# resibots/limbo

Measured on AMD Instinct MI355X. Metric: GP compute()+log_lik evaluations/sec at N=4096 D=6 fp64, higher is better.
Workload: dtype f64

## Files before the change

### limbo_amd/csrc/gemm.hip

```cpp
#include "dev.h"
#include <hip/hip_ext.h>
#include <cstdio>
#include <cstdint>
#include <cstdlib>
#include <map>
#include <mutex>
#include <tuple>
#include <vector>
#include <algorithm>

#ifdef GEMM_TIMING
__device__ long long g_gemm_ts[16];
#define GTS(i) do { if (threadIdx.x == 0 && blockIdx.x == 0 && lwg == (int)blockIdx.x) g_gemm_ts[i] = clock64(); } while (0)
__device__ long long g_gemm64_ts[24];
#define GTS64(i) do { if (threadIdx.x == 0 && blockIdx.x == 0 && lwg == (int)blockIdx.x) g_gemm64_ts[i] = clock64(); } while (0)
#else
#define GTS(i) do { } while (0)
#define GTS64(i) do { } while (0)
#endif
#ifdef GEMM_TIMING
#define GTS64_(i) GTS64(i)
#endif
#include "gemm_glds64.h"
#ifndef GEMM_ABL
// ... 127 lines not shown
    const double* Ap = AK ? g.A + kbeg + row0 * g.lda : g.A + row0 + kbeg * g.lda;
    const double* Bp = BK ? g.B + kbeg + col0 * g.ldb : g.B + col0 + kbeg * g.ldb;
    const int64_t a_kstep = AK ? (int64_t)BKT : (int64_t)BKT * g.lda;
    const int64_t b_kstep = BK ? (int64_t)BKT : (int64_t)BKT * g.ldb;
    const int64_t mrows = g.m - row0, ncols = g.n - col0;
    const int mr = (int)(mrows < TM ? mrows : TM), nc = (int)(ncols < TN ? ncols : TN);

    double acc[RA][RB];
#pragma unroll
    for (int a = 0; a < RA; ++a)
#pragma unroll
        for (int b = 0; b < RB; ++b)
            acc[a][b] = 0.0;

    using WT = WaveTileC<RA, RB>;
    double* Cw = g.C + (col0 + wn) * g.ldc + row0 + wm;
    const int rlim = mr - wm < WT::R ? mr - wm : WT::R, clim = nc - wn < WT::CN ? nc - wn : WT::CN;
    const bool live = rlim > 0 && clim > 0;
    constexpr bool CPRE = (NBUF == 1);
    double cv[WT::NIT];
    if (CPRE && live && g.overwrite != 1)
        WT::load(cv, Cw, g.ldc, rlim, clim, lane);

    SA sa;
    SB sb;
    int64_t kleft = kend - kbeg;
    if (kleft > 0) {
        const int kl = (int)(kleft < BKT ? kleft : BKT);
        sa.template load<true>(Ap, g.lda, mr, kl);
        sb.template load<false>(Bp, g.ldb, nc, kl);
        sa.store(lds[0]);
        sb.store(lds[0] + SA::ELEMS);
    }
    __syncthreads();
    int buf = 0;
    for (int64_t k0 = kbeg; k0 < kend; k0 += BKT) {
#if GEMM_ABL != 1
        const bool more = (NBUF == 2) && (k0 + BKT < kend);
#endif
#if GEMM_ABL == 1
        const bool more = false;
#endif
        if (more) {
            Ap += a_kstep;
            Bp += b_kstep;
            const int64_t kleft2 = kend - k0 - BKT;
            const int kl = (int)(kleft2 < BKT ? kleft2 : BKT);
            sa.template load<true>(Ap, g.lda, mr, kl);
            sb.template load<false>(Bp, g.ldb, nc, kl);
        }
        const double* As = lds[buf];
        const double* Bs = lds[buf] + SA::ELEMS;
#pragma unroll
        for (int ks = 0; ks < BKT; ks += 4) {
            double af[RA], bf[RB];
#pragma unroll
            for (int x = 0; x < RA; ++x)
                af[x] = SA::at(As, arow + 16 * x, ks + kq);
#pragma unroll
            for (int x = 0; x < RB; ++x)
                bf[x] = SB::at(Bs, bcol + 4 * x, ks + kq);
#pragma unroll
            for (int n = 0; n < RB; ++n)
#pragma unroll
                for (int m = 0; m < RA; ++m)
#if GEMM_ABL == 2
                    acc[m][n] += af[m] * bf[n] * (ks == 0 && m == 0 && n == 0 ? 1.0 : 0.0);
#else
                    acc[m][n] = mfma4(af[m], bf[n], acc[m][n]);
#endif
        }
        if (NBUF == 2) {
            if (more) {
                sa.store(lds[buf ^ 1]);
                sb.store(lds[buf ^ 1] + SA::ELEMS);
            }
            __syncthreads();
            buf ^= 1;
        }
    }

    static_assert(4 * WT::SCRATCH <= NBUF * (SA::ELEMS + SB::ELEMS), "transposition scratch must fit in the operand stages");
    if (!CPRE && live && g.overwrite != 1)
        WT::load(cv, Cw, g.ldc, rlim, clim, lane);
    if (NBUF == 1)
        __syncthreads();
    if (live)
        WT::store(acc, cv, &lds[0][0] + wave * WT::SCRATCH, Cw, g.ldc, rlim, clim, g.overwrite, lane);
}

template <typename K>
static void launch_k_named(const char* name, K kern_single, K kern_batched, dim3 grid, dim3 block, hipStream_t s, const GemmArgs& g0)
{
    GemmArgs g = g0;
    g.bt = g_batch.bt;
    grid.z = (unsigned)g_batch.G;
    K kern = g.bt ? kern_batched : kern_single;
    if (g.stop_event)
        GPE_LAUNCH_STOP(name, kern, grid, block, 0, s, (hipEvent_t)g.stop_event, g);
    else
        GPE_LAUNCH_NAMED(name, kern, grid, block, 0, s, g);
}
#define launch_k(ks, ...) launch_k_named(#ks, ks, __VA_ARGS__)
template <int TM, int TN, int BKT, int NBUF>
static void launch_tile(hipStream_t s, const GemmArgs& g0)
{
    GemmArgs g = g0;
    const int tiles_m = (int)((g.m + TM - 1) / TM), tiles_n = (int)((g.n + TN - 1) / TN);
    int64_t tiles = (int64_t)tiles_m * tiles_n;
    if (g.tri) {
        int fold = 1;
        const int nsup = (tiles_n + 1) / 2;
        for (int sc = 0; sc < nsup; ++sc) {
            const int t2 = tiles_n - 1 - sc;
            int len = tiles_m - first_live_tile<TM, TN>(g, sc);
            if (t2 != sc)
                len += tiles_m - first_live_tile<TM, TN>(g, t2);
            fold = len > fold ? len : fold;
        }
        g.fold_len = fold;
        tiles = (int64_t)nsup * fold;
    }
    dim3 grid((unsigned)tiles), block(256);
    if (!g.a_kmajor && !g.b_kmajor)
        launch_k(k_gemm4<TM, TN, BKT, NBUF, false, false>, k_gemm4<TM, TN, BKT, NBUF, false, false, true>, grid, block, s, g);
    else if (!g.a_kmajor && g.b_kmajor)
        launch_k(k_gemm4<TM, TN, BKT, NBUF, false, true>, k_gemm4<TM, TN, BKT, NBUF, false, true, true>, grid, block, s, g);
    else if (g.a_kmajor && !g.b_kmajor)
        launch_k(k_gemm4<TM, TN, BKT, NBUF, true, false>, k_gemm4<TM, TN, BKT, NBUF, true, false, true>, grid, block, s, g);
    else
        launch_k(k_gemm4<TM, TN, BKT, NBUF, true, true>, k_gemm4<TM, TN, BKT, NBUF, true, true, true>, grid, block, s, g);
}


template <int TM, int TN, int WM, int WN, int BKT, int NST, int EPC = 0, int MINB = 1, bool BATCH = false>
__global__ __launch_bounds__(WM* WN * 64, MINB) void k_gemm_glds(GemmArgs g_)
{
    GemmArgs gb;
    if (BATCH) {
        gb = g_;
        gemm_rebase(gb);
    }
    const GemmArgs& g = BATCH ? gb : g_;
    static_assert(TM == 128 && TN == 128, "one k-row of an operand tile = one 1 KiB glds instruction");
    constexpr int NWV = WM * WN;
    constexpr int SA = TM + 16, SB = TN + 16;
    constexpr int STAGE = BKT * (SA + SB);
    constexpr int RA = TM / WM / 16, RB = TN / WN / 4;
    constexpr int LPW = 2 * BKT / NWV;
    __shared__ __attribute__((aligned(16))) double lds[NST * STAGE];

    const int tiles_m = (int)((g.m + TM - 1) / TM);
    const int tiles_n = (int)((g.n + TN - 1) / TN);
    if (g.rhs_rows > 0)
        gemm_rhs_rows<64 * NWV, MINB == 1>(g, g.rhs_rows, (int)gridDim.x, lds);
    for (int lwg = blockIdx.x; lwg < g.total; lwg += gridDim.x) {
    int wg = lwg;
    {
        const int nwg = g.total;
        const int q = nwg / 8, r = nwg % 8, xcd = wg % 8, idx = wg / 8;
        wg = (xcd < r ? xcd * (q + 1) : r * (q + 1) + (xcd - r) * q) + idx;
    }
    int ti, tj;
    if (g.tile_map) {
        const int pk = g.tile_map[lwg];
        if (pk < 0)
            continue;
        ti = pk & 0xffff;
        tj = pk >> 16;
    }
    else if (g.tri) {
        const int sc = wg / g.fold_len;
        int rr = wg % g.fold_len;
        const int t0 = first_live_tile<TM, TN>(g, sc), c0 = tiles_m - t0;
        if (rr < c0) {
            tj = sc;
            ti = t0 + rr;
        }
        else {
            tj = tiles_n - 1 - sc;
            const int t1 = first_live_tile<TM, TN>(g, tj);
            rr -= c0;
            if (tj == sc || rr >= tiles_m - t1)
                continue;
            ti = t1 + rr;
        }
    }
    else {
        ti = wg % tiles_m;
        tj = wg / tiles_m;
    }
    const int64_t row0 = (int64_t)ti * TM, col0 = (int64_t)tj * TN;
    const int64_t mrows = g.m - row0, ncols = g.n - col0;
    const int mr = (int)(mrows < TM ? mrows : TM), nc = (int)(ncols < TN ? ncols : TN);

    const int lane = threadIdx.x & 63;
    const int wave = __builtin_amdgcn_readfirstlane(threadIdx.x >> 6);
    const int wm = (wave % WM) * (TM / WM), wn = (wave / WM) * (TN / WN);
    const int arow = wm + (lane & 15), bcol = wn + (lane & 3), kq = lane >> 4;

    int ra = 2 * lane, rb = 2 * lane;
    {
        const int ma = (mr - 1) & ~1, mb = (nc - 1) & ~1;
        ra = ra < ma ? ra : ma;
        rb = rb < mb ? rb : mb;
    }
    const int64_t kbeg = g.ktri ? (row0 > col0 ? row0 : col0) : 0;
    const double* pa = g.A + row0 + ra + ((int64_t)wave + kbeg) * g.lda;
    const double* pb = g.B + col0 + rb + ((int64_t)wave + kbeg) * g.ldb;
    const int64_t astep = (int64_t)NWV * g.lda, bstep = (int64_t)NWV * g.ldb;

    auto issue = [&](int stage) {
        double* sa = lds + stage * STAGE + wave * SA;
        double* sb = lds + stage * STAGE + BKT * SA + wave * SB;
#pragma unroll
        for (int q = 0; q < BKT / NWV; ++q) {
            __builtin_amdgcn_global_load_lds(pa, (lds_void_t*)(sa + q * NWV * SA), 16, 0, 0);
            __builtin_amdgcn_global_load_lds(pb, (lds_void_t*)(sb + q * NWV * SB), 16, 0, 0);
            pa += astep;
            pb += bstep;
        }
    };

    double acc[RA][RB];
#pragma unroll
    for (int a = 0; a < RA; ++a)
#pragma unroll
        for (int b = 0; b < RB; ++b)
            acc[a][b] = 0.0;

    const int nk = (int)((g.k - kbeg) / BKT);
    GTS(0);
    issue(0);
    for (int t = 0; t < nk; ++t) {
        const int st = t % NST;
        if (t + 1 < nk) {
            issue((t + 1) % NST);
            asm volatile("s_waitcnt vmcnt(%0)" ::"n"(LPW) : "memory");
        }
        else
            asm volatile("s_waitcnt vmcnt(0)" ::: "memory");
        __builtin_amdgcn_s_barrier();
        if (t == 0)
            GTS(1);
        if (t == 1)
            GTS(2);
        if (t == 2)
            GTS(3);
        const double* As = lds + st * STAGE;
        const double* Bs = As + BKT * SA;
#pragma unroll
        for (int ks = 0; ks < BKT; ks += 4) {
            double af[RA], bf[RB];
#pragma unroll
            for (int x = 0; x < RA; ++x)
                af[x] = As[(ks + kq) * SA + arow + 16 * x];
#pragma unroll
            for (int x = 0; x < RB; ++x)
                bf[x] = Bs[(ks + kq) * SB + bcol + 4 * x];
#pragma unroll
            for (int n = 0; n < RB; ++n)
#pragma unroll
                for (int m = 0; m < RA; ++m)
                    acc[m][n] = mfma4(af[m], bf[n], acc[m][n]);
        }
        if (t == 1)
            GTS(6);
        asm volatile("s_waitcnt lgkmcnt(0)" ::: "memory");
        __builtin_amdgcn_s_barrier();
        if (t == 1)
            GTS(7);
    }
    GTS(4);

    {
        using WT = WaveTileC<RA, RB>;
        constexpr int SCR = EPC > 0 ? WT::SCRATCH / EPC : WT::SCRATCH;
        static_assert(NWV * SCR <= NST * STAGE, "transposition scratch must fit in the operand stages");
        double* Cw = g.C + (col0 + wn) * g.ldc + row0 + wm;
        const int rlim = mr - wm < WT::R ? mr - wm : WT::R, clim = nc - wn < WT::CN ? nc - wn : WT::CN;
        if (rlim > 0 && clim > 0) {
            if constexpr (EPC > 0)
                WT::template rmw_chunked<EPC>(acc, lds + wave * SCR, Cw, g.ldc, rlim, clim, g.overwrite, lane);
            else {
                double cv[WT::NIT];
                if (g.overwrite != 1)
                    WT::load(cv, Cw, g.ldc, rlim, clim, lane);
                WT::store(acc, cv, lds + wave * WT::SCRATCH, Cw, g.ldc, rlim, clim, g.overwrite, lane);
            }
        }
    }
    __syncthreads();
    GTS(5);
    }
}
#ifdef GEMM_TIMING
void dump_gemm_timing()
{
    {
        long long q[24];
        (void)hipMemcpyFromSymbol(q, HIP_SYMBOL(g_gemm64_ts), sizeof(q));
        printf("k_gemm_glds64 WG0 first tile, cycles: start->k-tile 0 begins %lld | k-tiles:", q[1] - q[0]);
        for (int t = 1; t < 16; ++t)
            printf(" %lld", q[1 + t] - q[t]);
        printf(" %lld | epilogue %lld | total %lld\n", q[17] - q[16], q[18] - q[17], q[18] - q[0]);
    }
    long long h[16];
    (void)hipMemcpyFromSymbol(h, HIP_SYMBOL(g_gemm_ts), sizeof(h));
    printf("k_gemm_glds WG0 first tile, cycles: prologue (first stage landed) %lld | k-tile 0 %lld | k-tile 1 %lld (mfma part %lld, closing barrier %lld) | whole k loop %lld | epilogue %lld | total %lld\n",
           h[1] - h[0], h[2] - h[1], h[3] - h[2], h[6] - h[2], h[7] - h[6], h[4] - h[1], h[5] - h[4], h[5] - h[0]);
    printf("  epilogue: issue 32 loads %lld | loads complete %lld | issue 32 stores %lld | stores complete %lld | tail %lld\n", h[8] - h[4],
           h[9] - h[8], h[10] - h[9], h[11] - h[10], h[5] - h[11]);
}
#endif

template <int BKT, int NST, int MINB, int NWV, bool BATCH = false>
__global__ __launch_bounds__(64 * NWV, MINB) void k_gemm_glds64(GemmArgs g_)
{
    GemmArgs gb;
    if (BATCH) {
        gb = g_;
        gemm_rebase(gb);
    }
    const GemmArgs& g = BATCH ? gb : g_;
    __shared__ __attribute__((aligned(16))) double lds[NST * Glds64Shape<BKT>::STAGE];
    gemm_glds64_body<BKT, NST, NWV>(g, lds, (int)blockIdx.x, (int)gridDim.x, false);
}

static void launch_glds64(hipStream_t s, const GemmArgs& g0)
{
    constexpr int TM = 64, TN = 64;
    GemmArgs g = g0;
    const int tiles_m = (int)((g.m + TM - 1) / TM), tiles_n = (int)((g.n + TN - 1) / TN);
    int64_t tiles = (int64_t)tiles_m * tiles_n;
    if (g.tri) {
        int fold = 1;
        const int nsup = (tiles_n + 1) / 2;
        for (int sc = 0; sc < nsup; ++sc) {
            const int t2 = tiles_n - 1 - sc;
            int len = tiles_m - first_live_tile<TM, TN>(g, sc);
            if (t2 != sc)
                len += tiles_m - first_live_tile<TM, TN>(g, t2);
            fold = len > fold ? len : fold;
        }
        g.fold_len = fold;
        tiles = (int64_t)nsup * fold;
    }
    g.total = (int)tiles;
    if ((int64_t)g.total * g_batch.G > 256)
        launch_k(k_gemm_glds64<16, 4, 2, 4>, k_gemm_glds64<16, 4, 2, 4, true>, dim3((unsigned)tiles), dim3(256), s, g);
    else
        launch_k(k_gemm_glds64<16, 4, 1, 8>, k_gemm_glds64<16, 4, 1, 8, true>, dim3((unsigned)tiles), dim3(512), s, g);
}

static bool glds_ok(const GemmArgs& g)
{
    return !g.a_kmajor && !g.b_kmajor && !g.ktri && g.k >= 32 && g.k % 32 == 0 && (g.lda % 2) == 0 && (g.ldb % 2) == 0
        && ((uintptr_t)g.A % 16) == 0 && ((uintptr_t)g.B % 16) == 0;
}

#define TRI_BAND 8
struct TriMapKey {
    int dev, tiles_m, tiles_n;
    int64_t off;
    bool operator<(const TriMapKey& o) const
    {
        return std::tie(dev, tiles_m, tiles_n, off) < std::tie(o.dev, o.tiles_m, o.tiles_n, o.off);
    }
};
static int tri_tile_map_host(const GemmArgs& g, std::vector<int>& tab)
{
    constexpr int TM = 128, TN = 128;
    const int tiles_m = (int)((g.m + TM - 1) / TM), tiles_n = (int)((g.n + TN - 1) / TN);
    std::vector<int> first(tiles_n);
    for (int tj = 0; tj < tiles_n; ++tj)
        first[tj] = first_live_tile<TM, TN>(g, tj);
    std::vector<int> seq;
    for (int r0 = 0; r0 < tiles_m; r0 += TRI_BAND) {
        const int r1 = std::min(tiles_m, r0 + TRI_BAND);
        for (int tj = 0; tj < tiles_n; ++tj)
            for (int ti = std::max(r0, first[tj]); ti < r1; ++ti)
                seq.push_back(ti | (tj << 16));
    }
    const int T = (int)seq.size(), q = T / 8, r = T % 8, slots = q + (r ? 1 : 0);
    tab.assign((size_t)slots * 8, -1);
    int pos = 0;
    for (int x = 0; x < 8; ++x) {
        const int len = q + (x < r ? 1 : 0);
        for (int i = 0; i < len; ++i)
            tab[(size_t)i * 8 + x] = seq[pos + i];
        pos += len;
    }
    return (int)tab.size();
}
int debug_tri_tile_map(int64_t m, int64_t n, int64_t grow0, int64_t gcol0, int* out, int cap)
{
    GemmArgs g{};
    g.m = m;
    g.n = n;
    g.tri = 1;
    g.grow0 = grow0;
    g.gcol0 = gcol0;
    std::vector<int> tab;
    const int len = tri_tile_map_host(g, tab);
    for (int i = 0; i < len && i < cap; ++i)
        out[i] = tab[i];
    return len;
}
static const int* tri_tile_map(const GemmArgs& g, int* total)
{
    static std::mutex mu;
    static std::map<TriMapKey, std::pair<int*, int>> cache;
    int dev = 0;
    (void)hipGetDevice(&dev);
    const TriMapKey key{dev, (int)((g.m + 127) / 128), (int)((g.n + 127) / 128), g.gcol0 - g.grow0};
    std::lock_guard<std::mutex> lk(mu);
    auto it = cache.find(key);
    if (it == cache.end()) {
        std::vector<int> tab;
        const int len = tri_tile_map_host(g, tab);
        int* d = nullptr;
        if (hipMalloc(&d, sizeof(int) * (size_t)len) != hipSuccess)
            return nullptr;
        if (hipMemcpy(d, tab.data(), sizeof(int) * (size_t)len, hipMemcpyHostToDevice) != hipSuccess) {
            (void)hipFree(d);
            return nullptr;
// ... 408 lines not shown
```

### limbo_amd/csrc/potrf_tail.hip

```cpp
#include "potrf_tile.h"
#include <array>
#include <map>
#include <mutex>
#include <vector>
#ifdef DIAG_TIMING
__device__ long long g_tail_ts[64][4];
__device__ long long g_tail_cyc[64][4];
#define TTS(c, i) do { if (threadIdx.x == 0 && (c) < 64) { g_tail_ts[(c)][(i)] = wall_clock64(); g_tail_cyc[(c)][(i)] = clock64(); } } while (0)
__device__ long long g_tail_ts2[64][12];
#define TTS2(x, on, i) do { if ((on) && threadIdx.x == 0 && ((x).R0 - (x).p0) / NB < 64) g_tail_ts2[((x).R0 - (x).p0) / NB][(i)] = wall_clock64(); } while (0)
#else
#define TTS(c, i) do { } while (0)
#define TTS2(x, on, i) do { } while (0)
#endif

struct TailArgs {
    double* A;
    int64_t lda, t0;
    int nt, nb;
    int nfull;
    int rhs_rows;
    double* Xt;
    int* info;
    double *LP, *SP, *LPn, *SPn;
// ... 348 lines not shown
    }
    __syncthreads();
    TTS2(x, true, 3);
    double y2[2][2] = {{0.0, 0.0}, {0.0, 0.0}};
    tri_solve32(T, 32, X22, wm, hn, lane, y2);
#pragma unroll
    for (int m = 0; m < 2; ++m)
#pragma unroll
        for (int n = 0; n < 2; ++n)
            Ys[(hn + 4 * n + dcol) * PS + wm + 16 * m + drow] = y2[m][n];
    __syncthreads();
    TTS2(x, true, 4);
    syrk40<32>(Ys, 0, wave, lane, a2v);
    syrk40_store_neg(Dl, wave, lane, a2v);
    {
        const int i = threadIdx.x & 63, kk0 = threadIdx.x >> 6;
#pragma unroll
        for (int q = 0; q < 4; ++q) {
            const int col = kk0 + 8 * q;
            __hip_atomic_store(pub + i + NB * (32 + col), Ys[col * PS + i], __ATOMIC_RELAXED, __HIP_MEMORY_SCOPE_AGENT);
        }
    }
#pragma unroll
    for (int m = 0; m < 2; ++m)
#pragma unroll
        for (int n = 0; n < 2; ++n)
            T[(32 + hn + 4 * n + dcol) * PS + wm + 16 * m + drow] = y2[m][n];
    TTS2(x, true, 5);
}

static __device__ __forceinline__ void tail_tile_solve(const P256& x, double* __restrict__ lds, const double (&own)[8],
                                                       const double* __restrict__ Sq, double* __restrict__ pub, const bool near)
{
    const int lane = threadIdx.x & 63, wave = __builtin_amdgcn_readfirstlane(threadIdx.x >> 6);
    const int wm = (wave & 1) * 32, wn = (wave >> 1) * 16;
    const int hn = tri_solve_cols(wave);
    const int crow = wm + (lane & 31), ccol = wn + (lane >> 5);
    const int drow = 4 * ((lane >> 2) & 3) + (lane >> 4), dcol = lane & 3;
    double* const T = lds + CH_T;
    double* const X11 = lds + CH_X11;
    double* const Ld = lds + CH_LD;
    double* const Ys = lds + CH_YS;
    double* const X22 = lds + CH_X22;
    const unsigned long long SENT = ~0ull;
    const unsigned long long* Sp = reinterpret_cast<const unsigned long long*>(Sq) + threadIdx.x;
#pragma unroll
    for (int it = 0; it < 8; ++it)
        T[(ccol + 2 * it) * PS + crow] = own[it];
    {
        unsigned long long xb[4];
#pragma unroll
        for (int q = 0; q < 4; ++q)
            xb[q] = __hip_atomic_load(Sp + 512 * q, __ATOMIC_RELAXED, POLL_FIRST_SCOPE);
        if (near)
            chain_watch<4>(Sp, xb, x.spin_limit, x.info);
        else {
            int spins = 0;
            while (xb[0] == SENT || xb[1] == SENT || xb[2] == SENT || xb[3] == SENT) {
                if (++spins > x.spin_limit) {
                    x.info[2] = 1;
                    break;
                }
                poll_one(Sq + 1023, x.spin_limit, x.info);
                poll_one(Sq + 1024 + 32 * 31, x.spin_limit, x.info);
#pragma unroll
                for (int q = 0; q < 4; ++q)
                    if (xb[q] == SENT)
                        xb[q] = __hip_atomic_load(Sp + 512 * q, __ATOMIC_RELAXED, __HIP_MEMORY_SCOPE_AGENT);
            }
        }
#pragma unroll
        for (int q = 0; q < 2; ++q) {
            const int e = threadIdx.x + 512 * q;
            X11[(e >> 5) * 34 + (e & 31)] = __longlong_as_double((long long)xb[q]);
            Ld[(e & 31) * 34 + (e >> 5)] = __longlong_as_double((long long)xb[2 + q]);
        }
    }
    __syncthreads();
    double y1[2][2] = {{0.0, 0.0}, {0.0, 0.0}};
    tri_solve32(T, 0, X11, wm, hn, lane, y1);
#pragma unroll
    for (int m = 0; m < 2; ++m)
#pragma unroll
        for (int n = 0; n < 2; ++n)
            Ys[(hn + 4 * n + dcol) * PS + wm + 16 * m + drow] = y1[m][n];
    __syncthreads();
    double u[2][2] = {{0.0, 0.0}, {0.0, 0.0}};
    mmk<true, 32, 2, 34>(Ys, 0, Ld, 0, wm, hn, lane, u);
#pragma unroll
    for (int m = 0; m < 2; ++m)
#pragma unroll
        for (int n = 0; n < 2; ++n) {
            double* t = T + (32 + hn + 4 * n + dcol) * PS + wm + 16 * m + drow;
            *t = *t - u[m][n];
            T[(hn + 4 * n + dcol) * PS + wm + 16 * m + drow] = y1[m][n];
        }
    {
        const int i = threadIdx.x & 63, kk0 = threadIdx.x >> 6;
#pragma unroll
        for (int q = 0; q < 4; ++q) {
            const int col = kk0 + 8 * q;
            __hip_atomic_store(pub + i + NB * col, Ys[col * PS + i], __ATOMIC_RELAXED, __HIP_MEMORY_SCOPE_AGENT);
        }
    }
    {
        unsigned long long xc[2];
        xc[0] = __hip_atomic_load(Sp + 2048, __ATOMIC_RELAXED, POLL_FIRST_SCOPE);
        xc[1] = __hip_atomic_load(Sp + 2048 + 512, __ATOMIC_RELAXED, POLL_FIRST_SCOPE);
        if (near)
            chain_watch<2>(Sp + 2048, xc, x.spin_limit, x.info);
        else {
            int spins = 0;
            while (xc[0] == SENT || xc[1] == SENT) {
                if (++spins > x.spin_limit) {
                    x.info[2] = 1;
                    break;
                }
                poll_one(Sq + 2048 + 1023, x.spin_limit, x.info);
                if (xc[0] == SENT)
                    xc[0] = __hip_atomic_load(Sp + 2048, __ATOMIC_RELAXED, __HIP_MEMORY_SCOPE_AGENT);
                if (xc[1] == SENT)
                    xc[1] = __hip_atomic_load(Sp + 2048 + 512, __ATOMIC_RELAXED, __HIP_MEMORY_SCOPE_AGENT);
            }
        }
        const int e0 = threadIdx.x, e1 = threadIdx.x + 512;
        X22[(e0 >> 5) * 34 + (e0 & 31)] = __longlong_as_double((long long)xc[0]);
        X22[(e1 >> 5) * 34 + (e1 & 31)] = __longlong_as_double((long long)xc[1]);
    }
    __syncthreads();
    double y2[2][2] = {{0.0, 0.0}, {0.0, 0.0}};
    tri_solve32(T, 32, X22, wm, hn, lane, y2);
#pragma unroll
    for (int m = 0; m < 2; ++m)
#pragma unroll
        for (int n = 0; n < 2; ++n)
            Ys[(hn + 4 * n + dcol) * PS + wm + 16 * m + drow] = y2[m][n];
    __syncthreads();
    {
        const int i = threadIdx.x & 63, kk0 = threadIdx.x >> 6;
#pragma unroll
        for (int q = 0; q < 4; ++q) {
            const int col = kk0 + 8 * q;
            __hip_atomic_store(pub + i + NB * (32 + col), Ys[col * PS + i], __ATOMIC_RELAXED, __HIP_MEMORY_SCOPE_AGENT);
        }
    }
#pragma unroll
    for (int m = 0; m < 2; ++m)
#pragma unroll
        for (int n = 0; n < 2; ++n)
            T[(32 + hn + 4 * n + dcol) * PS + wm + 16 * m + drow] = y2[m][n];
    __syncthreads();
}

static __device__ __forceinline__ void tail_body(const TailArgs& a, const int wgid, double* __restrict__ lds,
                                                 const KParams* __restrict__ kp = nullptr)
{
    const int lane = threadIdx.x & 63, wave = __builtin_amdgcn_readfirstlane(threadIdx.x >> 6);
    const int wm = (wave & 1) * 32, wn = (wave >> 1) * 16;
    const int crow = wm + (lane & 31), ccol = wn + (lane >> 5);
    int c = 0, b;
    if (a.order) {
        b = __builtin_amdgcn_readfirstlane(a.order[2 * wgid]);
        c = __builtin_amdgcn_readfirstlane(a.order[2 * wgid + 1]);
    }
    else {
        int id = wgid, colh = a.nb;
        while (id >= colh) {
            id -= colh;
            ++c;
            --colh;
        }
        b = c + id;
    }
    const int slot = tail_tile_id(a.nb, b, c);
    const bool mute = a.spin_limit < 0;
    P256 x;
    x.A = a.A;
    x.lda = a.lda;
    x.p0 = a.t0;
    x.R0 = a.t0 + (int64_t)NB * b;
    x.Xt = a.Xt;
    x.info = a.info;
    x.mute = mute;
    x.spin_limit = mute ? -a.spin_limit : a.spin_limit;
    x.nrows = b < a.nfull ? NB : a.rhs_rows;
    x.want_d = false;
    x.Bx = lds;
    x.T0 = lds + NB * XS;
    x.T1 = x.T0 + NB * PS;
    x.T2 = x.T1 + NB * PS;
    x.S22 = a.SP;
    x.HP = a.LP;
    double* const myslot = a.LP + (int64_t)slot * (NB * NB);
    {
        unsigned long long* nx = reinterpret_cast<unsigned long long*>(a.LPn + (int64_t)slot * (NB * NB));
#pragma unroll
        for (int q = 0; q < 8; ++q)
            nx[threadIdx.x + 512 * q] = ~0ull;
        if (b == c) {
            unsigned long long* ns = reinterpret_cast<unsigned long long*>(a.SPn + (int64_t)c * 3072);
#pragma unroll
            for (int q = 0; q < 6; ++q)
                ns[threadIdx.x + 512 * q] = ~0ull;
        }
    }
    if (b == c + 1 && b < a.nt)
        return;
    const int crc = crow < x.nrows ? crow : x.nrows - 1;
    double cv[8];
    if (kp) {
        tail_gen_tile(a, kp, x.R0 + crc, a.t0 + (int64_t)NB * c + ccol, cv);
        if (a.Al && b >= a.nfull && threadIdx.x < NB)
            for (int p = 0; p < a.P; ++p)
                reinterpret_cast<unsigned long long*>(a.Al)[a.t0 + (int64_t)NB * c + threadIdx.x + (int64_t)p * a.ldal] = ~0ull;
    }
    else {
#pragma unroll
        for (int it = 0; it < 8; ++it)
            cv[it] = a.A[x.R0 + crc + (a.t0 + (int64_t)NB * c + ccol + 2 * it) * a.lda];
    }
    if (b == c) {
        double* const Dl = lds + CH_D;
        double* const Ltb = lds + CH_AUX;
        double* const invd = Ltb + DIAG_LTB;
        DiagSync* const sy = reinterpret_cast<DiagSync*>(invd + NB);
        if (c > 0) {
            double cl[8];
            if (kp)
                tail_gen_tile(a, kp, x.R0 + crow, a.t0 + (int64_t)NB * (c - 1) + ccol, cl);
            else {
#pragma unroll
                for (int it = 0; it < 8; ++it)
                    cl[it] = a.A[x.R0 + crow + (a.t0 + (int64_t)NB * (c - 1) + ccol + 2 * it) * a.lda];
            }
            tail_chain_updates_and_crossing(a, x, lds, c, cl, cv);
            TTS(c, 1);
        }
        else {
#pragma unroll
            for (int it = 0; it < 8; ++it)
                Dl[crow * XS + ccol + 2 * it] = cv[it];
            diag_flow_init(sy);
        }
        __syncthreads();
        DiagEarly ea;
        ea.mute = mute;
        ea.S = a.SP + (int64_t)c * 3072;
        TTS(c, 2);
        diag_flow(Dl, Ltb, invd, sy, a.A + x.R0 + x.R0 * a.lda, a.lda, a.Xt + (int64_t)c * (NB * NB), a.info, x.R0, wave, lane,
                  invd + NB + 8, &ea);
        TTS(c, 3);
        if (c > 0) {
            __syncthreads();
            const int i = threadIdx.x & 63, kk0 = threadIdx.x >> 6;
            double* Ag = a.A + x.R0 + (a.t0 + (int64_t)NB * (c - 1)) * a.lda;
            const double* T = lds + CH_T;
#pragma unroll
            for (int q = 0; q < 8; ++q) {
                const int col = kk0 + 8 * q;
                Ag[i + (int64_t)col * a.lda] = T[col * PS + i];
            }
        }
        return;
    }
    PolledTile pa, pb;
    if (c > 0) {
        pa.issue(a.LP + (int64_t)tail_tile_id(a.nb, b, 0) * (NB * NB));
        pb.issue(a.LP + (int64_t)tail_tile_id(a.nb, c, 0) * (NB * NB));
    }
    double a2[2][4] = {{0.0, 0.0, 0.0, 0.0}, {0.0, 0.0, 0.0, 0.0}};
#pragma unroll 1
    for (int s = 0; s < c; ++s) {
        double* const opA = lds + (s & 1) * (2 * NB * PS);
        double* const opB = opA + NB * PS;
        pa.finish(a.LP + (int64_t)tail_tile_id(a.nb, b, s) * (NB * NB), x.spin_limit, x.info);
        pa.store(opA);
        pb.finish(a.LP + (int64_t)tail_tile_id(a.nb, c, s) * (NB * NB), x.spin_limit, x.info);
        pb.store(opB);
        if (s + 1 < c) {
            pa.issue(a.LP + (int64_t)tail_tile_id(a.nb, b, s + 1) * (NB * NB));
            pb.issue(a.LP + (int64_t)tail_tile_id(a.nb, c, s + 1) * (NB * NB));
        }
        __syncthreads();
        mm64<false>(opA, opB, wm, wn, lane, a2);
    }
    if (c > 0) {
        double a2r[8];
        wave_tile_to_rows(a2, a2r, lane);
#pragma unroll
        for (int it = 0; it < 8; ++it)
            cv[it] -= a2r[it];
        __syncthreads();
    }
    tail_tile_solve(x, lds, cv, a.SP + (int64_t)c * 3072, myslot, b - c <= 3);
    {
        const int i = threadIdx.x & 63, kk0 = threadIdx.x >> 6;
        double* Ag = a.A + x.R0 + (a.t0 + (int64_t)NB * c) * a.lda;
        const double* T = lds + CH_T;
        if (i < x.nrows) {
#pragma unroll
            for (int q = 0; q < 8; ++q) {
                const int col = kk0 + 8 * q;
                Ag[i + (int64_t)col * a.lda] = T[col * PS + i];
            }
        }
    }
}

__global__ __launch_bounds__(512) void k_tail(TailArgs a)
{
    __shared__ __attribute__((aligned(16))) double lds[TAIL_LDS_DOUBLES];
    tail_body(a, (int)blockIdx.x, lds);
}
__global__ __launch_bounds__(512) void k_tail_g(TailArgs a, KParams kp)
{
    __shared__ __attribute__((aligned(16))) double lds[TAIL_LDS_DOUBLES];
    tail_body(a, (int)blockIdx.x, lds, &kp);
}
__global__ __launch_bounds__(512) void k_tail_b(TailArgs a, const BatchTab* __restrict__ bt)
{
    __shared__ __attribute__((aligned(16))) double lds[TAIL_LDS_DOUBLES];
    const int G = bt->G, gp = (int)blockIdx.x % G;
    a.A = bt_rebase(bt, gp, a.A);
    a.Xt = bt_rebase(bt, gp, a.Xt);
    a.info = bt_rebase(bt, gp, a.info);
    a.LP = bt_rebase(bt, gp, a.LP);
    a.SP = bt_rebase(bt, gp, a.SP);
    a.LPn = bt_rebase(bt, gp, a.LPn);
    a.SPn = bt_rebase(bt, gp, a.SPn);
    if (a.Xg) {
        a.Xg = bt_rebase(bt, gp, a.Xg);
        a.Om = bt_rebase(bt, gp, a.Om);
        a.Al = bt_rebase(bt, gp, a.Al);
    }
    tail_body(a, (int)blockIdx.x / G, lds, a.Xg ? &bt->kp[gp] : nullptr);
}

__global__ __launch_bounds__(256) void k_ragged_partial(const double* __restrict__ A, int64_t ld, int m, int n, int64_t k, int kc,
                                                        double* __restrict__ part)
{
    __shared__ __attribute__((aligned(16))) double As[32][NB];
    const int li = threadIdx.x & 63, lk = threadIdx.x >> 6;
    const int ti = threadIdx.x & 15, tj = threadIdx.x >> 4;
    const int64_t k0 = (int64_t)blockIdx.x * kc, k1 = k0 + kc < k ? k0 + kc : k;
    double acc[4][4];
#pragma unroll
    for (int r = 0; r < 4; ++r)
#pragma unroll
        for (int c = 0; c < 4; ++c)
            acc[r][c] = 0.0;
    double nx[8];
    auto fetch = [&](int64_t kb) {
#pragma unroll
        for (int q = 0; q < 8; ++q) {
            const int kk = lk + 4 * q;
            nx[q] = (kb + kk < k1 && li < m) ? A[li + (kb + kk) * ld] : 0.0;
        }
    };
    fetch(k0);
    for (int64_t kb = k0; kb < k1; kb += 32) {
        __syncthreads();
#pragma unroll
        for (int q = 0; q < 8; ++q)
            As[lk + 4 * q][li] = nx[q];
        if (kb + 32 < k1)
            fetch(kb + 32);
        __syncthreads();
#pragma unroll 8
        for (int kk = 0; kk < 32; ++kk) {
            double a[4], b[4];
#pragma unroll
            for (int r = 0; r < 4; ++r) {
                a[r] = As[kk][4 * ti + r];
                b[r] = As[kk][4 * tj + r];
            }
#pragma unroll
            for (int r = 0; r < 4; ++r)
#pragma unroll
                for (int c = 0; c < 4; ++c)
                    acc[r][c] = fma(a[r], b[c], acc[r][c]);
        }
    }
    double* out = part + (int64_t)blockIdx.x * (NB * NB);
#pragma unroll
    for (int c = 0; c < 4; ++c)
#pragma unroll
        for (int r = 0; r < 4; ++r)
            out[4 * ti + r + NB * (4 * tj + c)] = acc[r][c];
}
#define RAGGED_MAX_G 32
__global__ __launch_bounds__(256) void k_ragged_fold(double* __restrict__ C, int64_t ldc, int m, int n, int G, const double* __restrict__ part)
{
    const int i = threadIdx.x & 63, j = 4 * (int)blockIdx.x + (threadIdx.x >> 6);
    if (i >= m || j >= n || i < j)
        return;
    double v[RAGGED_MAX_G];
#pragma unroll
    for (int g = 0; g < RAGGED_MAX_G; ++g)
        v[g] = g < G ? part[(int64_t)g * (NB * NB) + i + NB * j] : 0.0;
    double sum = 0.0;
#pragma unroll
    for (int g = 0; g < RAGGED_MAX_G; ++g)
        sum += v[g];
    C[i + (int64_t)j * ldc] -= sum;
}
int ragged_split(int64_t k, int64_t scratch_doubles, int* kc_out)
{
    if (k < 256 || scratch_doubles < 2 * NB * NB)
        return 0;
    int64_t G = k / 64;
    G = G > RAGGED_MAX_G ? RAGGED_MAX_G : G;
    G = G > scratch_doubles / (NB * NB) ? scratch_doubles / (NB * NB) : G;
    const int64_t kc = ((k + G - 1) / G + 31) / 32 * 32;
    G = (k + kc - 1) / kc;
    *kc_out = (int)kc;
    return (int)G;
}
__global__ __launch_bounds__(DIAG_THREADS) void k_ragged_finish(double* __restrict__ C, int64_t ldc, int jb, int P, int G,
                                                                const double* __restrict__ part, double* __restrict__ Lscr,
                                                                double* __restrict__ Xt, int* __restrict__ info, int64_t goff)
{
    __shared__ __attribute__((aligned(16))) double Ls[NB * XS];
    __shared__ __attribute__((aligned(16))) double Ltb[DIAG_LTB];
    __shared__ __attribute__((aligned(16))) double invd[NB];
    __shared__ DiagSync sy;
    __shared__ __attribute__((aligned(16))) double Xw[DIAG_XW_DOUBLES];
    __shared__ double Rr[NB * 65];
    const int lane = threadIdx.x & 63, w = __builtin_amdgcn_readfirstlane(threadIdx.x >> 6);
    const int m = jb + P;
    for (int e = threadIdx.x; e < NB * 65; e += DIAG_THREADS)
// ... 282 lines not shown
```

### limbo_amd/csrc/sweep2.hip

```cpp
#include "gemm_glds64.h"

#define NB 64
#define S2_PS 80
#define S2_MS 65

#ifdef S2_TIMING
__device__ long long g_s2_ts[256][6];
#define S2TS(i) do { if (threadIdx.x == 0) g_s2_ts[j][i] = wall_clock64(); } while (0)
#else
#define S2TS(i) do { } while (0)
#endif

__global__ __launch_bounds__(512) void k_trsv_bwd_m(const double* __restrict__ L, int64_t ld, int64_t N, const double* __restrict__ Xt_all,
                                                    const double* __restrict__ y, int64_t ysi, double* a, int* __restrict__ err,
                                                    const double* __restrict__ om, double* __restrict__ part)
{
    __shared__ __attribute__((aligned(16))) double lds[2 * NB * S2_PS];
    __shared__ double Mt[NB * S2_MS], M2t[NB * S2_MS];
    __shared__ double xs[NB], wj[NB], gj[NB], part_s[8 * NB];
    const int lane = threadIdx.x & 63, wv = threadIdx.x >> 6;
    const int wvu = __builtin_amdgcn_readfirstlane(wv);
    const int64_t nblk = (N + NB - 1) / NB;
    const int64_t j = flow_block_of(nblk, true);
    if (j < 0)
        return;
    const int64_t j0 = j * NB;
    const int jb = (int)((N - j0 < NB) ? N - j0 : NB);
    const double* Xt = Xt_all + j * (NB * NB);
    const unsigned long long SENT = ~0ull;
    S2TS(0);
    if (j + 1 < nblk) {
        double* As = lds;
        double* Bs = lds + NB * S2_PS;
        const int wm = (wvu & 1) * 32, wn = (wvu >> 1) * 16;
        const int ar = wm + (lane & 15), bc = wn + (lane & 3), kq = lane >> 4;
        const int drow = 4 * ((lane >> 2) & 3) + (lane >> 4), dcol = lane & 3;
#pragma unroll
        for (int q = 0; q < 8; ++q) {
            const int r = wvu + 8 * q;
            As[r * S2_PS + lane] = Xt[lane + NB * r];
        }
        for (int q2 = 1; q2 <= 2 && j + q2 < nblk; ++q2) {
            const int64_t t0 = (j + q2) * NB;
            const int tb = (int)((N - t0 < NB) ? N - t0 : NB);
            const int kc = lane < tb ? lane : tb - 1;
            const double km = lane < tb ? 1.0 : 0.0;
            if (q2 == 2)
                __syncthreads();
#pragma unroll
            for (int q = 0; q < 8; ++q) {
                const int r = wvu + 8 * q;
                const int rc = r < jb ? r : jb - 1;
                Bs[r * S2_PS + lane] = L[t0 + kc + (j0 + rc) * ld] * (r < jb ? km : 0.0);
            }
            __syncthreads();
            double acc[2][4] = {{0.0, 0.0, 0.0, 0.0}, {0.0, 0.0, 0.0, 0.0}};
#pragma unroll
            for (int ks = 0; ks < NB; ks += 4) {
                double af[2], bf[4];
#pragma unroll
                for (int x = 0; x < 2; ++x)
                    af[x] = As[(ks + kq) * S2_PS + ar + 16 * x];
#pragma unroll
                for (int x = 0; x < 4; ++x)
                    bf[x] = Bs[(ks + kq) * S2_PS + bc + 4 * x];
#pragma unroll
                for (int n = 0; n < 4; ++n)
#pragma unroll
                    for (int m = 0; m < 2; ++m)
                        acc[m][n] = mfma4(af[m], bf[n], acc[m][n]);
            }
            double* Md = q2 == 1 ? Mt : M2t;
#pragma unroll
            for (int m = 0; m < 2; ++m)
#pragma unroll
                for (int n = 0; n < 4; ++n)
                    Md[(wn + 4 * n + dcol) * S2_MS + wm + 16 * m + drow] = acc[m][n];
        }
    }
    S2TS(1);
    double* Stg = lds;
    __syncthreads();
    if (threadIdx.x < NB)
        wj[lane] = (lane < jb) ? y[(j0 + lane) * ysi] : 0.0;
    double tl[4][8];
    unsigned long long pb[4] = {SENT, SENT, SENT, SENT};
    auto fetch = [&](double (&dst)[8], unsigned long long& peek, int64_t tt) {
        const int64_t t0 = tt * NB;
        const int tb = (int)((N - t0 < NB) ? N - t0 : NB);
        const int kc = lane < tb ? lane : tb - 1;
#pragma unroll
        for (int q = 0; q < 8; ++q) {
            const int c = wvu + 8 * q;
            const int cc = c < jb ? c : jb - 1;
            dst[q] = L[t0 + kc + (j0 + cc) * ld];
        }
        peek = __hip_atomic_load((const unsigned long long*)(a + t0 + kc), __ATOMIC_RELAXED, __HIP_MEMORY_SCOPE_AGENT);
    };
    auto await = [&](unsigned long long peek, int64_t t) {
        double v = 0.0;
        const int64_t t0 = t * NB;
        const int tb = (int)((N - t0 < NB) ? N - t0 : NB);
        if (lane < tb) {
            unsigned long long bits = peek;
            int spins = 0;
            while (bits == SENT) {
                if ((spins & 3) != 3)
                    bits = __hip_atomic_load((const unsigned long long*)(a + t0 + lane), __ATOMIC_RELAXED, __HIP_MEMORY_SCOPE_WORKGROUP);
                else
                    bits = __hip_atomic_load((const unsigned long long*)(a + t0 + lane), __ATOMIC_RELAXED, __HIP_MEMORY_SCOPE_AGENT);
                if (bits != SENT)
                    break;
                if (++spins > GPE_FLOW_SPIN_LIMIT) {
                    *err = 1;
                    break;
                }
                __builtin_amdgcn_s_sleep(1);
            }
            v = __longlong_as_double((long long)bits);
        }
        return v;
    };
    auto fold = [&](const double (&src)[8], unsigned long long peek, int64_t t) {
        __syncthreads();
        const int tbf = (int)((N - t * NB < NB) ? N - t * NB : NB);
        const double rowmask = lane < tbf ? 1.0 : 0.0;
#pragma unroll
        for (int q = 0; q < 8; ++q)
            Stg[(wv + 8 * q) * 65 + lane] = src[q] * (wvu + 8 * q < jb ? rowmask : 0.0);
        if (threadIdx.x < NB)
            xs[lane] = await(peek, t);
        __syncthreads();
        double acc = 0.0;
#pragma unroll
        for (int kk = 0; kk < 8; ++kk) {
            const int k = 8 * wv + kk;
            acc = fma(Stg[lane * 65 + k], xs[k], acc);
        }
        part_s[wv * NB + lane] = acc;
        __syncthreads();
        if (threadIdx.x < NB) {
            double s = part_s[lane];
#pragma unroll
            for (int w = 1; w < 8; ++w)
                s += part_s[w * NB + lane];
            wj[lane] -= s;
        }
    };
    const int64_t lo = j + 2;
    int64_t t = nblk - 1;
    auto clampt = [&](int64_t tt) { return tt > lo ? tt : (lo + 1 < nblk ? lo + 1 : nblk - 1); };
    if (t > lo) {
        fetch(tl[0], pb[0], clampt(t));
        fetch(tl[1], pb[1], clampt(t - 1));
        fetch(tl[2], pb[2], clampt(t - 2));
        fetch(tl[3], pb[3], clampt(t - 3));
    }
    for (; t - 3 > lo; t -= 4) {
        fold(tl[0], pb[0], t);
        fetch(tl[0], pb[0], clampt(t - 4));
        fold(tl[1], pb[1], t - 1);
        fetch(tl[1], pb[1], clampt(t - 5));
        fold(tl[2], pb[2], t - 2);
        fetch(tl[2], pb[2], clampt(t - 6));
        fold(tl[3], pb[3], t - 3);
        fetch(tl[3], pb[3], clampt(t - 7));
    }
    if (t > lo)
        fold(tl[0], pb[0], t);
    if (t - 1 > lo)
        fold(tl[1], pb[1], t - 1);
    if (t - 2 > lo)
        fold(tl[2], pb[2], t - 2);
    unsigned long long p2 = SENT, p1 = SENT;
    if (threadIdx.x < NB) {
        if (j + 2 < nblk) {
            const int64_t t0 = (j + 2) * NB;
            const int tb = (int)((N - t0 < NB) ? N - t0 : NB);
            p2 = __hip_atomic_load((const unsigned long long*)(a + t0 + (lane < tb ? lane : tb - 1)), __ATOMIC_RELAXED, __HIP_MEMORY_SCOPE_AGENT);
        }
        if (j + 1 < nblk) {
            const int64_t t0 = (j + 1) * NB;
            const int tb = (int)((N - t0 < NB) ? N - t0 : NB);
            p1 = __hip_atomic_load((const unsigned long long*)(a + t0 + (lane < tb ? lane : tb - 1)), __ATOMIC_RELAXED, __HIP_MEMORY_SCOPE_AGENT);
        }
    }
    __syncthreads();
    {
        double acc = 0.0;
#pragma unroll
        for (int kk = 0; kk < 8; ++kk) {
            const int r = 8 * wv + kk;
            acc = fma(Xt[lane + NB * r], wj[r], acc);
        }
        part_s[wv * NB + lane] = acc;
        __syncthreads();
        if (threadIdx.x < NB) {
            double s = part_s[lane];
#pragma unroll
            for (int w = 1; w < 8; ++w)
                s += part_s[w * NB + lane];
            gj[lane] = s;
        }
    }
    S2TS(2);
    auto step = [&](const double* Mx, unsigned long long peek, int64_t tt) {
        if (threadIdx.x < NB)
            xs[lane] = await(peek, tt);
        __syncthreads();
        double acc = 0.0;
#pragma unroll
        for (int kk = 0; kk < 8; ++kk) {
            const int k = 8 * wv + kk;
            acc = fma(Mx[k * S2_MS + lane], xs[k], acc);
        }
        part_s[wv * NB + lane] = acc;
        __syncthreads();
        double r = 0.0;
        if (threadIdx.x < NB) {
            double s = part_s[lane];
#pragma unroll
            for (int w = 1; w < 8; ++w)
                s += part_s[w * NB + lane];
            r = gj[lane] - s;
            gj[lane] = r;
        }
        return r;
    };
    double aj = 0.0;
    if (j + 2 < nblk)
        (void)step(M2t, p2, j + 2);
    S2TS(3);
    if (j + 1 < nblk)
        aj = step(Mt, p1, j + 1);
    else {
        __syncthreads();
        if (threadIdx.x < NB)
            aj = gj[lane];
    }
    if (threadIdx.x < NB) {
        if (lane < jb)
            __hip_atomic_store((unsigned long long*)(a + j0 + lane), (unsigned long long)__double_as_longlong(aj), __ATOMIC_RELAXED,
                               __HIP_MEMORY_SCOPE_AGENT);
        S2TS(4);
        if (part) {
            double ldp = lane < jb ? log(L[(j0 + lane) + (j0 + lane) * ld]) : 0.0;
            double oa = (om && lane < jb) ? om[j0 + lane] * aj : 0.0;
#pragma unroll
            for (int o = 32; o > 0; o >>= 1) {
                ldp += __shfl_xor(ldp, o);
                oa += __shfl_xor(oa, o);
            }
            if (lane == 0) {
                part[j] = ldp;
                part[nblk + j] = oa;
            }
        }
    }
}

#ifdef S2_TIMING
#include <cstdio>
void dump_s2_timing(int nblk)
{
    static long long h[256][6];
    (void)hipMemcpyFromSymbol(h, HIP_SYMBOL(g_s2_ts), sizeof(h));
    const long long t0 = h[nblk - 1][0];
    printf("backward sweep with M_j (us after the first workgroup started): block | start | M_j done | g_j ready | a_{j+1} seen | a_j published (hop)\n");
    for (int j = nblk - 1; j >= 0; --j)
        printf("  %3d | %6.2f | %6.2f | %6.2f | %6.2f | %6.2f (%5.2f)\n", j, (h[j][0] - t0) * 0.01, (h[j][1] - t0) * 0.01, (h[j][2] - t0) * 0.01,
               (h[j][3] - t0) * 0.01, (h[j][4] - t0) * 0.01, j + 1 < nblk ? (h[j][4] - h[j + 1][4]) * 0.01 : 0.0);
}
#endif

void launch_trsv_bwd_m(hipStream_t s, const double* L, int64_t ld, int64_t N, const double* Xt_all, const double* y, int64_t ysi, double* a,
                       int* err, int prefilled, const double* om, double* part)
{
    const int64_t nblk = (N + NB - 1) / NB;
    if (!prefilled)
        hipMemsetAsync(a, 0xFF, sizeof(double) * (size_t)N, s);
    FlowGate gate(s);
    GPE_LAUNCH(k_trsv_bwd_m, dim3(GPE_FLOW_GRID(nblk)), dim3(512), 0, s, L, ld, N, Xt_all, y, ysi, a, err, om, part);
}
```

Before: 948.8.

## Fuse right-hand-side rows into GEMM tiles, prefetch tail tiles, restructure sweep2 head

The GEMM kernel now computes up to four extra right-hand-side rows inside the first live tile of each column, loading them through a small LDS buffer, instead of running a separate rhs-rows pass. The potrf tail issues its polled tile loads earlier and skips the finish spin when the wave already holds the data. Sweep2 loads Xt and L into registers first, issues its fetches before the small MFMA precompute, and takes a direct path without that precompute for the last few blocks. Together these aim to cut latency and serialisation in the Cholesky and solve chain, at the cost of extra registers and more complex wait-count logic.

```diff
diff --git a/limbo_amd/csrc/gemm.hip b/limbo_amd/csrc/gemm.hip
--- a/limbo_amd/csrc/gemm.hip
+++ b/limbo_amd/csrc/gemm.hip
@@ -303,8 +303,19 @@
 
     const int tiles_m = (int)((g.m + TM - 1) / TM);
     const int tiles_n = (int)((g.n + TN - 1) / TN);
-    if (g.rhs_rows > 0)
-        gemm_rhs_rows<64 * NWV, MINB == 1>(g, g.rhs_rows, (int)gridDim.x, lds);
+    constexpr bool ROWS_IN_TILE = MINB == 1 && !BATCH && NWV == 8 && BKT == 32;
+    constexpr int ZST = 4 * BKT;
+    __shared__ __attribute__((aligned(16))) double zrow[ROWS_IN_TILE ? NST * ZST : 1];
+    bool rows_in_tile = false;
+    if constexpr (ROWS_IN_TILE) {
+        rows_in_tile = g.rhs_rows > 0 && g.rhs_rows <= 4 && !g.ktri && (!g.tri || first_live_tile<TM, TN>(g, tiles_n - 1) < tiles_m);
+        if (g.rhs_rows > 0 && !rows_in_tile)
+            gemm_rhs_rows<64 * NWV, MINB == 1>(g, g.rhs_rows, (int)gridDim.x, lds);
+    }
+    else {
+        if (g.rhs_rows > 0)
+            gemm_rhs_rows<64 * NWV, MINB == 1>(g, g.rhs_rows, (int)gridDim.x, lds);
+    }
     for (int lwg = blockIdx.x; lwg < g.total; lwg += gridDim.x) {
     int wg = lwg;
     {
@@ -360,10 +371,20 @@
     const double* pa = g.A + row0 + ra + ((int64_t)wave + kbeg) * g.lda;
     const double* pb = g.B + col0 + rb + ((int64_t)wave + kbeg) * g.ldb;
     const int64_t astep = (int64_t)NWV * g.lda, bstep = (int64_t)NWV * g.ldb;
+    const bool rows_here = rows_in_tile && ti == (g.tri ? first_live_tile<TM, TN>(g, tj) : 0);
+    const bool zwave = rows_here && wave < g.rhs_rows;
+    const char* pz = reinterpret_cast<const char*>(g.A + g.m + (zwave ? wave : 0) + (kbeg + (lane >> 1)) * g.lda) + 4 * (lane & 1);
+    const int64_t zstep = (int64_t)BKT * g.lda * 8;
 
     auto issue = [&](int stage) {
         double* sa = lds + stage * STAGE + wave * SA;
         double* sb = lds + stage * STAGE + BKT * SA + wave * SB;
+        if constexpr (ROWS_IN_TILE) {
+            if (zwave) {
+                __builtin_amdgcn_global_load_lds(pz, (lds_void_t*)(zrow + stage * ZST + wave * BKT), 4, 0, 0);
+                pz += zstep;
+            }
+        }
 #pragma unroll
         for (int q = 0; q < BKT / NWV; ++q) {
             __builtin_amdgcn_global_load_lds(pa, (lds_void_t*)(sa + q * NWV * SA), 16, 0, 0);
@@ -372,6 +393,7 @@
             pb += bstep;
         }
     };
+    double racc[4] = {0.0, 0.0, 0.0, 0.0};
 
     double acc[RA][RB];
 #pragma unroll
@@ -387,7 +409,10 @@
         const int st = t % NST;
         if (t + 1 < nk) {
             issue((t + 1) % NST);
-            asm volatile("s_waitcnt vmcnt(%0)" ::"n"(LPW) : "memory");
+            if (ROWS_IN_TILE && zwave)
+                asm volatile("s_waitcnt vmcnt(%0)" ::"n"(LPW + 1) : "memory");
+            else
+                asm volatile("s_waitcnt vmcnt(%0)" ::"n"(LPW) : "memory");
         }
         else
             asm volatile("s_waitcnt vmcnt(0)" ::: "memory");
@@ -400,6 +425,18 @@
             GTS(3);
         const double* As = lds + st * STAGE;
         const double* Bs = As + BKT * SA;
+        double rbv[8], rzv[8];
+        if constexpr (ROWS_IN_TILE) {
+            if (rows_here) {
+                const double* Zs = zrow + st * ZST + (threadIdx.x >> 7) * 8;
+                const double* Bc = Bs + (threadIdx.x >> 7) * 8 * SB + (threadIdx.x & 127);
+#pragma unroll
+                for (int i = 0; i < 8; ++i) {
+                    rbv[i] = Bc[i * SB];
+                    rzv[i] = Zs[i];
+                }
+            }
+        }
 #pragma unroll
         for (int ks = 0; ks < BKT; ks += 4) {
             double af[RA], bf[RB];
@@ -414,6 +451,25 @@
 #pragma unroll
                 for (int m = 0; m < RA; ++m)
                     acc[m][n] = mfma4(af[m], bf[n], acc[m][n]);
+        }
+        if constexpr (ROWS_IN_TILE) {
+            if (rows_here) {
+                const double* Zs = zrow + st * ZST + (threadIdx.x >> 7) * 8;
+                const int np = g.rhs_rows;
+#pragma unroll
+                for (int i = 0; i < 8; ++i)
+                    racc[0] = fma(rzv[i], rbv[i], racc[0]);
+#pragma unroll
+                for (int p = 1; p < 4; ++p)
+                    if (p < np) {
+#pragma unroll
+                        for (int i = 0; i < 8; ++i)
+                            rzv[i] = Zs[p * BKT + i];
+#pragma unroll
+                        for (int i = 0; i < 8; ++i)
+                            racc[p] = fma(rzv[i], rbv[i], racc[p]);
+                    }
+            }
         }
         if (t == 1)
             GTS(6);
@@ -423,6 +479,22 @@
             GTS(7);
     }
     GTS(4);
+
+    if constexpr (ROWS_IN_TILE) {
+        if (rows_here) {
+            const int c = threadIdx.x & 127, kg = threadIdx.x >> 7, np = g.rhs_rows;
+#pragma unroll
+            for (int p = 0; p < 4; ++p)
+                lds[(p * 4 + kg) * 128 + c] = racc[p];
+            __syncthreads();
+            if (kg < np && c < nc) {
+                double* Cp = g.C + (g.m + kg) + (col0 + c) * g.ldc;
+                const double* rp = lds + kg * 4 * 128 + c;
+                *Cp = *Cp - (((rp[0] + rp[128]) + rp[256]) + rp[384]);
+            }
+            __syncthreads();
+        }
+    }
 
     {
         using WT = WaveTileC<RA, RB>;
diff --git a/limbo_amd/csrc/potrf_tail.hip b/limbo_amd/csrc/potrf_tail.hip
--- a/limbo_amd/csrc/potrf_tail.hip
+++ b/limbo_amd/csrc/potrf_tail.hip
@@ -524,6 +524,15 @@
     __syncthreads();
 }
 
+static __device__ __forceinline__ void polled_finish(PolledTile& p, const double* G, int spin_limit, int* __restrict__ info)
+{
+    const unsigned long long SENT = ~0ull;
+    const bool pending = p.b[0] == SENT || p.b[1] == SENT || p.b[2] == SENT || p.b[3] == SENT || p.b[4] == SENT || p.b[5] == SENT
+        || p.b[6] == SENT || p.b[7] == SENT;
+    if (__builtin_amdgcn_ballot_w64(pending) != 0)
+        p.finish(G, spin_limit, info);
+}
+
 static __device__ __forceinline__ void tail_body(const TailArgs& a, const int wgid, double* __restrict__ lds,
                                                  const KParams* __restrict__ kp = nullptr)
 {
@@ -564,6 +573,12 @@
     x.S22 = a.SP;
     x.HP = a.LP;
     double* const myslot = a.LP + (int64_t)slot * (NB * NB);
+    const bool looks_first = c > 0 && b != c && !(b == c + 1 && b < a.nt);
+    PolledTile pa, pb;
+    if (looks_first) {
+        pa.issue(a.LP + (int64_t)tail_tile_id(a.nb, b, 0) * (NB * NB));
+        pb.issue(a.LP + (int64_t)tail_tile_id(a.nb, c, 0) * (NB * NB));
+    }
     {
         unsigned long long* nx = reinterpret_cast<unsigned long long*>(a.LPn + (int64_t)slot * (NB * NB));
 #pragma unroll
@@ -635,19 +650,14 @@
         }
         return;
     }
-    PolledTile pa, pb;
-    if (c > 0) {
-        pa.issue(a.LP + (int64_t)tail_tile_id(a.nb, b, 0) * (NB * NB));
-        pb.issue(a.LP + (int64_t)tail_tile_id(a.nb, c, 0) * (NB * NB));
-    }
     double a2[2][4] = {{0.0, 0.0, 0.0, 0.0}, {0.0, 0.0, 0.0, 0.0}};
 #pragma unroll 1
     for (int s = 0; s < c; ++s) {
         double* const opA = lds + (s & 1) * (2 * NB * PS);
         double* const opB = opA + NB * PS;
-        pa.finish(a.LP + (int64_t)tail_tile_id(a.nb, b, s) * (NB * NB), x.spin_limit, x.info);
+        polled_finish(pa, a.LP + (int64_t)tail_tile_id(a.nb, b, s) * (NB * NB), x.spin_limit, x.info);
         pa.store(opA);
-        pb.finish(a.LP + (int64_t)tail_tile_id(a.nb, c, s) * (NB * NB), x.spin_limit, x.info);
+        polled_finish(pb, a.LP + (int64_t)tail_tile_id(a.nb, c, s) * (NB * NB), x.spin_limit, x.info);
         pb.store(opB);
         if (s + 1 < c) {
             pa.issue(a.LP + (int64_t)tail_tile_id(a.nb, b, s + 1) * (NB * NB));
diff --git a/limbo_amd/csrc/sweep2.hip b/limbo_amd/csrc/sweep2.hip
--- a/limbo_amd/csrc/sweep2.hip
+++ b/limbo_amd/csrc/sweep2.hip
@@ -3,6 +3,7 @@
 #define NB 64
 #define S2_PS 80
 #define S2_MS 65
+#define S2_HEAD 8
 
 #ifdef S2_TIMING
 __device__ long long g_s2_ts[256][6];
@@ -28,61 +29,28 @@
     const int jb = (int)((N - j0 < NB) ? N - j0 : NB);
     const double* Xt = Xt_all + j * (NB * NB);
     const unsigned long long SENT = ~0ull;
+    const bool direct = j + S2_HEAD >= nblk;
     S2TS(0);
-    if (j + 1 < nblk) {
-        double* As = lds;
-        double* Bs = lds + NB * S2_PS;
-        const int wm = (wvu & 1) * 32, wn = (wvu >> 1) * 16;
-        const int ar = wm + (lane & 15), bc = wn + (lane & 3), kq = lane >> 4;
-        const int drow = 4 * ((lane >> 2) & 3) + (lane >> 4), dcol = lane & 3;
-#pragma unroll
-        for (int q = 0; q < 8; ++q) {
-            const int r = wvu + 8 * q;
-            As[r * S2_PS + lane] = Xt[lane + NB * r];
-        }
-        for (int q2 = 1; q2 <= 2 && j + q2 < nblk; ++q2) {
-            const int64_t t0 = (j + q2) * NB;
+    double xr[8];
+#pragma unroll
+    for (int q = 0; q < 8; ++q)
+        xr[q] = Xt[lane + NB * (wvu + 8 * q)];
+    const bool mpath = j + 1 < nblk && !direct;
+    double lm[2][8];
+    if (mpath) {
+#pragma unroll
+        for (int q2 = 1; q2 <= 2; ++q2) {
+            const int64_t tq = j + q2 < nblk ? j + q2 : nblk - 1;
+            const int64_t t0 = tq * NB;
             const int tb = (int)((N - t0 < NB) ? N - t0 : NB);
             const int kc = lane < tb ? lane : tb - 1;
-            const double km = lane < tb ? 1.0 : 0.0;
-            if (q2 == 2)
-                __syncthreads();
 #pragma unroll
             for (int q = 0; q < 8; ++q) {
                 const int r = wvu + 8 * q;
-                const int rc = r < jb ? r : jb - 1;
-                Bs[r * S2_PS + lane] = L[t0 + kc + (j0 + rc) * ld] * (r < jb ? km : 0.0);
-            }
-            __syncthreads();
-            double acc[2][4] = {{0.0, 0.0, 0.0, 0.0}, {0.0, 0.0, 0.0, 0.0}};
-#pragma unroll
-            for (int ks = 0; ks < NB; ks += 4) {
-                double af[2], bf[4];
-#pragma unroll
-                for (int x = 0; x < 2; ++x)
-                    af[x] = As[(ks + kq) * S2_PS + ar + 16 * x];
-#pragma unroll
-                for (int x = 0; x < 4; ++x)
-                    bf[x] = Bs[(ks + kq) * S2_PS + bc + 4 * x];
-#pragma unroll
-                for (int n = 0; n < 4; ++n)
-#pragma unroll
-                    for (int m = 0; m < 2; ++m)
-                        acc[m][n] = mfma4(af[m], bf[n], acc[m][n]);
-            }
-            double* Md = q2 == 1 ? Mt : M2t;
-#pragma unroll
-            for (int m = 0; m < 2; ++m)
-#pragma unroll
-                for (int n = 0; n < 4; ++n)
-                    Md[(wn + 4 * n + dcol) * S2_MS + wm + 16 * m + drow] = acc[m][n];
-        }
-    }
-    S2TS(1);
-    double* Stg = lds;
-    __syncthreads();
-    if (threadIdx.x < NB)
-        wj[lane] = (lane < jb) ? y[(j0 + lane) * ysi] : 0.0;
+                lm[q2 - 1][q] = L[t0 + kc + (j0 + (r < jb ? r : jb - 1)) * ld];
+            }
+        }
+    }
     double tl[4][8];
     unsigned long long pb[4] = {SENT, SENT, SENT, SENT};
     auto fetch = [&](double (&dst)[8], unsigned long long& peek, int64_t tt) {
@@ -97,6 +65,67 @@
         }
         peek = __hip_atomic_load((const unsigned long long*)(a + t0 + kc), __ATOMIC_RELAXED, __HIP_MEMORY_SCOPE_AGENT);
     };
+    const int64_t lo = direct ? j : j + 2;
+    int64_t t = nblk - 1;
+    auto clampt = [&](int64_t tt) { return tt > lo ? tt : (lo + 1 < nblk ? lo + 1 : nblk - 1); };
+    if (t > lo) {
+        fetch(tl[0], pb[0], clampt(t));
+        fetch(tl[1], pb[1], clampt(t - 1));
+        fetch(tl[2], pb[2], clampt(t - 2));
+        fetch(tl[3], pb[3], clampt(t - 3));
+    }
+    if (mpath) {
+        double* As = lds;
+        double* Bs = lds + NB * S2_PS;
+        const int wm = (wvu & 1) * 32, wn = (wvu >> 1) * 16;
+        const int ar = wm + (lane & 15), bc = wn + (lane & 3), kq = lane >> 4;
+        const int drow = 4 * ((lane >> 2) & 3) + (lane >> 4), dcol = lane & 3;
+#pragma unroll
+        for (int q = 0; q < 8; ++q) {
+            const int r = wvu + 8 * q;
+            As[r * S2_PS + lane] = xr[q];
+        }
+        for (int q2 = 1; q2 <= 2 && j + q2 < nblk; ++q2) {
+            const int64_t t0 = (j + q2) * NB;
+            const int tb = (int)((N - t0 < NB) ? N - t0 : NB);
+            const double km = lane < tb ? 1.0 : 0.0;
+            if (q2 == 2)
+                __syncthreads();
+#pragma unroll
+            for (int q = 0; q < 8; ++q) {
+                const int r = wvu + 8 * q;
+                Bs[r * S2_PS + lane] = lm[q2 - 1][q] * (r < jb ? km : 0.0);
+            }
+            __syncthreads();
+            double acc[2][4] = {{0.0, 0.0, 0.0, 0.0}, {0.0, 0.0, 0.0, 0.0}};
+#pragma unroll
+            for (int ks = 0; ks < NB; ks += 4) {
+                double af[2], bf[4];
+#pragma unroll
+                for (int x = 0; x < 2; ++x)
+                    af[x] = As[(ks + kq) * S2_PS + ar + 16 * x];
+#pragma unroll
+                for (int x = 0; x < 4; ++x)
+                    bf[x] = Bs[(ks + kq) * S2_PS + bc + 4 * x];
+#pragma unroll
+                for (int n = 0; n < 4; ++n)
+#pragma unroll
+                    for (int m = 0; m < 2; ++m)
+                        acc[m][n] = mfma4(af[m], bf[n], acc[m][n]);
+            }
+            double* Md = q2 == 1 ? Mt : M2t;
+#pragma unroll
+            for (int m = 0; m < 2; ++m)
+#pragma unroll
+                for (int n = 0; n < 4; ++n)
+                    Md[(wn + 4 * n + dcol) * S2_MS + wm + 16 * m + drow] = acc[m][n];
+        }
+    }
+    S2TS(1);
+    double* Stg = lds;
+    __syncthreads();
+    if (threadIdx.x < NB)
+        wj[lane] = (lane < jb) ? y[(j0 + lane) * ysi] : 0.0;
     auto await = [&](unsigned long long peek, int64_t t) {
         double v = 0.0;
         const int64_t t0 = t * NB;
@@ -147,15 +176,6 @@
             wj[lane] -= s;
         }
     };
-    const int64_t lo = j + 2;
-    int64_t t = nblk - 1;
-    auto clampt = [&](int64_t tt) { return tt > lo ? tt : (lo + 1 < nblk ? lo + 1 : nblk - 1); };
-    if (t > lo) {
-        fetch(tl[0], pb[0], clampt(t));
-        fetch(tl[1], pb[1], clampt(t - 1));
-        fetch(tl[2], pb[2], clampt(t - 2));
-        fetch(tl[3], pb[3], clampt(t - 3));
-    }
     for (; t - 3 > lo; t -= 4) {
         fold(tl[0], pb[0], t);
         fetch(tl[0], pb[0], clampt(t - 4));
@@ -173,7 +193,7 @@
     if (t - 2 > lo)
         fold(tl[2], pb[2], t - 2);
     unsigned long long p2 = SENT, p1 = SENT;
-    if (threadIdx.x < NB) {
+    if (threadIdx.x < NB && !direct) {
         if (j + 2 < nblk) {
             const int64_t t0 = (j + 2) * NB;
             const int tb = (int)((N - t0 < NB) ? N - t0 : NB);
@@ -190,8 +210,8 @@
         double acc = 0.0;
 #pragma unroll
         for (int kk = 0; kk < 8; ++kk) {
-            const int r = 8 * wv + kk;
-            acc = fma(Xt[lane + NB * r], wj[r], acc);
+            const int r = wv + 8 * kk;
+            acc = fma(xr[kk], wj[r], acc);
         }
         part_s[wv * NB + lane] = acc;
         __syncthreads();
@@ -228,10 +248,10 @@
         return r;
     };
     double aj = 0.0;
-    if (j + 2 < nblk)
+    if (j + 2 < nblk && !direct)
         (void)step(M2t, p2, j + 2);
     S2TS(3);
-    if (j + 1 < nblk)
+    if (j + 1 < nblk && !direct)
         aj = step(Mt, p1, j + 1);
     else {
         __syncthreads();
```

New measurement: 957.7 (median of 6 runs). No clear change (+0.9%).
